# dkogan/libdogleg

Hardware: AMD Instinct MI355X
Metric: trust-region steps/sec (fp64) at fixed (Nmeas,Nstate,nnz) (higher is better)
Workload: dtype f64

## Files before the change

include/dlg_backend.h:

```cpp
#ifndef DLG_BACKEND_H
#define DLG_BACKEND_H

#include <stddef.h>

#ifdef __cplusplus
extern "C" {
#endif

typedef struct dlg_backend dlg_backend_t;

enum
{
  DLG_OK           = 0,
  DLG_ERR_HIP      = 1,
  DLG_ERR_ARG      = 2,
  DLG_ERR_STATE    = 3,
  DLG_ERR_NOMEM    = 4,
  DLG_ERR_NODEVICE = 5,
  DLG_ERR_COMM     = 6
};

enum { DLG_DENSE = 0, DLG_SPARSE = 1, DLG_DENSE_PRODUCTS = 2 };
enum { DLG_FLAG_JTJ_PACKED = 1, DLG_FLAG_JTJ_UPPER = 2 };
enum { DLG_KIND_CAUCHY_TO_EDGE = 0, DLG_KIND_GAUSSNEWTON = 1, DLG_KIND_INTERPOLATED = 2 };
// ... 21 lines not shown
int  dlg_partition_rows(dlg_backend_t* b, int* nrows, const int** rows);
int  dlg_point_gather_device(dlg_backend_t* b, int slot, const double* x_full_dev, const double* J_full_dev,
                             const int* colptr_host);
int  dlg_partition_stats(dlg_backend_t* b, long* stats, int nstats);
int  dlg_sparse_partition_probe(int N, int M, const int* colptr, const int* rowidx, int rank, int nranks,
                                long* stats, int nstats, char* row_owner);
int  dlg_rccl_unique_id(void* out128);
int  dlg_backend_init_rccl(dlg_backend_t* b, int rank, int nranks, const void* unique_id128);
int  dlg_backend_set_rccl(dlg_backend_t* b, void* nccl_comm);
int  dlg_backend_share_rccl(dlg_backend_t* b, dlg_backend_t* owner);
int  dlg_backend_comm_size(dlg_backend_t* b, int* nranks);
int  dlg_backend_has_rccl(dlg_backend_t* b);
int  dlg_backend_set_noop_comm(dlg_backend_t* b, int on);

int  dlg_run_steps(dlg_backend_t* b, int from, int to, int nsteps, int ncopy, const double* const* x_dev,
                   const double* const* J_dev, int first_copy, double trustregion, double lambda0,
                   double* out9, int* kind_out);

int  dlg_backend_reset(dlg_backend_t* b);
int  dlg_backend_device(dlg_backend_t* b);
int  dlg_sparse_pattern_matches(dlg_backend_t* b, const int* colptr, const int* rowidx);
int  dlg_sparse_drop_pattern(dlg_backend_t* b);

int  dlg_sparse_set_pattern(dlg_backend_t* b, const int* colptr, const int* rowidx);
int  dlg_sparse_stats(dlg_backend_t* b, long* nnz_JtJ_lower, long* nnz_L,
                      int* n_supernodes, int* n_levels, double* factor_flops);

int  dlg_sparse_region_probe(int N, int M, const int* colptr, const int* rowidx, int ncu, long* stats, int nstats);

int  dlg_sparse_schedule(dlg_backend_t* b, int* n_levels, int* persist_level0, int* persist_items);

int  dlg_sparse_leaf_rows_stats(dlg_backend_t* b, long* stats, int nstats);

int  dlg_sparse_symbolic_probe(int N, int M, const int* colptr, const int* rowidx, int row0,
                               int row1, long* stats, int nstats, int* perm_out);

int  dlg_point_set_p(dlg_backend_t* b, int slot, const double* p_host);
int  dlg_point_upload(dlg_backend_t* b, int slot, const double* x_host,
                      const double* J_host);
int  dlg_point_upload_products(dlg_backend_t* b, int slot, double norm2x,
                               const double* Jtx_host, const double* JtJ_host);
int  dlg_point_bind_device(dlg_backend_t* b, int slot, const double* x_dev,
                           const double* J_dev);
int  dlg_point_eval(dlg_backend_t* b, int slot, double* norm2_x, double* Jtx_absmax);
int  dlg_backend_set_speculation(dlg_backend_t* b, int on);
typedef void (*dlg_between_fn)(void* cookie);
int  dlg_backend_set_between(dlg_backend_t* b, dlg_between_fn fn, void* cookie);
int  dlg_backend_between_redone(dlg_backend_t* b);
int  dlg_point_eval_early(dlg_backend_t* b, int slot, const double* x_dev, const double* J_dev, int* done);
int  dlg_backend_set_defer_tail(dlg_backend_t* b, int on);
int  dlg_step_tail_pending(dlg_backend_t* b);
int  dlg_backend_ei_source(dlg_backend_t* b, int* from_solved_system, double* pivot_ratio);
int  dlg_step_tail(dlg_backend_t* b, double* expected_improvement);
int  dlg_backend_time_allreduce(dlg_backend_t* b, size_t count, int iters, double* us_each);

int  dlg_cauchy(dlg_backend_t* b, int slot, double* norm2_updateCauchy);

int  dlg_factorize(dlg_backend_t* b, int slot, double lambda, int* ok);

int  dlg_solve_gn(dlg_backend_t* b, int slot, double* norm2_updateGN);

int  dlg_gauss_newton(dlg_backend_t* b, int slot, double* lambda_io, double* norm2_updateGN);

int  dlg_cauchy_gauss_newton(dlg_backend_t* b, int slot, double* lambda_io, double* norm2_updateCauchy,
                             double* norm2_updateGN);

// ... 88 lines not shown
```

libdogleg_amd/capi.py:

```python
import ctypes as C
import os
import numpy as np

from .ctypes_defs import (Parameters2, CholmodSparse, Trace, TraceBuffer, BatchResult, BatchLoss, BatchBounds, JacobianReport, JacobianEntry,
                          CB_SPARSE, CB_DENSE, CB_PRODUCTS, dptr, iptr)

HERE = os.path.dirname(os.path.abspath(__file__))
LIB_PATH = os.environ.get("DLG_TEST_LIB") or os.path.join(HERE, "libdogleg_amd.so")

DLG_OK = 0
DLG_DENSE, DLG_SPARSE, DLG_DENSE_PRODUCTS = 0, 1, 2
FLAG_PACKED, FLAG_UPPER = 1, 2
KIND_CAUCHY, KIND_GN, KIND_INTERP = 0, 1, 2
VEC_P, VEC_X, VEC_JTX, VEC_CAUCHY, VEC_GN, VEC_STEP, VEC_J, VEC_X_OWN, VEC_J_OWN = range(9)

ALLREDUCE_FN = C.CFUNCTYPE(C.c_int, C.c_void_p, C.c_size_t, C.c_void_p)

BACKEND_SYMBOLS = [
    "dlg_last_error", "dlg_device_count", "dlg_backend_create", "dlg_backend_destroy",
    "dlg_backend_set_stream", "dlg_backend_get_stream", "dlg_backend_set_shard",
    "dlg_sparse_set_pattern", "dlg_sparse_stats", "dlg_sparse_schedule", "dlg_sparse_leaf_rows_stats", "dlg_point_set_p", "dlg_point_upload",
    "dlg_point_upload_products", "dlg_point_bind_device", "dlg_point_eval", "dlg_cauchy",
    "dlg_factorize", "dlg_solve_gn", "dlg_gauss_newton", "dlg_cauchy_gauss_newton", "dlg_make_step",
    "dlg_expected_improvement", "dlg_step", "dlg_take_step", "dlg_solve_with_factor",
    "dlg_point_download", "dlg_factor_download_dense", "dlg_point_device_ptr",
    "dlg_kernel_syrk_lower", "dlg_kernel_potrf_lower", "dlg_probe_mfma_f64", "dlg_probe_mfma_f64_clock", "dlg_probe_mfma_f64_waves",
    "dlg_probe_hbm_copy", "dlg_set_trace", "dlg_mem_alloc", "dlg_mem_free", "dlg_host_alloc",
    "dlg_host_free", "dlg_mem_upload",
    "dlg_mem_download", "dlg_mem_zero", "dlg_device_sync", "dlg_sparse_symbolic_probe",
    "dlg_backend_set_profiling", "dlg_backend_get_profile", "dlg_backend_get_profile_early",
    "dlg_backend_set_allreduce", "dlg_backend_set_partition", "dlg_partition_rows", "dlg_partition_stats",
    "dlg_sparse_partition_probe", "dlg_rccl_unique_id", "dlg_backend_init_rccl", "dlg_backend_set_rccl",
    "dlg_backend_comm_size", "dlg_backend_has_rccl", "dlg_backend_set_noop_comm", "dlg_solve_multi", "dlg_pseudoinverse_chunk", "dlg_backend_set_speculation", "dlg_backend_set_defer_tail", "dlg_step_tail",
    "dlg_step_tail_pending", "dlg_backend_ei_source", "dlg_backend_set_between", "dlg_backend_between_redone", "dlg_point_eval_early",
    "dlg_backend_share_rccl", "dlg_point_gather_device", "dlg_backend_reset", "dlg_backend_device",
    "dlg_sparse_pattern_matches", "dlg_sparse_drop_pattern", "dlg_sparse_region_probe", "dlg_run_steps", "dlg_backend_time_allreduce",
    "dlg_feature_leverage", "dlg_outlierness_factors", "dlg_leverage_query", "dlg_leverage_stats",
    "dlg_covariance_blocks", "dlg_marginal_variances", "dlg_covariance_stats", "dlg_covariance_plan_seconds",
    "dlg_covariance_plan_probe", "dlg_covariance_entries", "dlg_covariance_entries_stats", "dlg_covariance_entries_probe",
    "dlg_query_covariance", "dlg_query_covariance_stats", "dlg_query_covariance_plan_seconds", "dlg_query_covariance_plan_probe",
]
PROF_NAMES = ["K1_jtx", "K3K8_norm2Jv", "K4_kernel", "K4_total", "K5_factor", "K6_solve", "K7_step", "vec"]
DOGLEG_SYMBOLS = [
    "dogleg_getDefaultParameters", "dogleg_setMaxIterations",
    "dogleg_setTrustregionUpdateParameters", "dogleg_setDebug", "dogleg_setInitialTrustregion",
    "dogleg_setThresholds", "dogleg_optimize", "dogleg_optimize2", "dogleg_optimize_dense",
    "dogleg_optimize_dense2", "dogleg_optimize_dense_products", "dogleg_computeJtJfactorization",
    "dogleg_freeContext", "dogleg_testGradient", "dogleg_testGradient_dense",
    "dogleg_testGradient_dense_products",
    "dogleg_optimize_device2", "dogleg_amd_backend", "dogleg_amd_point_slot",
    "dogleg_amd_set_communicator", "dogleg_amd_set_allreduce", "dogleg_amd_clear_communicator",
    "dogleg_amd_rccl_unique_id", "dogleg_amd_rank", "dogleg_amd_release_cache",
    "dogleg_amd_id_file_publish", "dogleg_amd_id_file_wait", "dogleg_amd_last_solve_timing",
    "dogleg_getOutliernessFactors", "dogleg_markOutliers", "dogleg_reportOutliers",
# ... 30 lines not shown
                       "g.build()'` (there is no CPU fallback)")
    L = C.CDLL(LIB_PATH)
    D, I, V = C.POINTER(C.c_double), C.POINTER(C.c_int), C.c_void_p
    L.dlg_last_error.restype = C.c_char_p
    L.dlg_device_count.restype = C.c_int
    L.dlg_backend_create.argtypes = [C.POINTER(V), C.c_int, C.c_int, C.c_int, C.c_int, C.c_int, C.c_int]
    L.dlg_backend_destroy.argtypes = [V]
    L.dlg_backend_destroy.restype = None
    L.dlg_backend_set_stream.argtypes = [V, V]
    L.dlg_backend_get_stream.argtypes = [V]
    L.dlg_backend_get_stream.restype = V
    L.dlg_backend_set_shard.argtypes = [V, C.c_int, C.c_int, V, V]
    L.dlg_backend_set_allreduce.argtypes = [V, V, V]
    L.dlg_backend_set_speculation.argtypes = [V, C.c_int]
    L.dlg_backend_set_defer_tail.argtypes = [V, C.c_int]
    L.dlg_step_tail.argtypes = [V, C.POINTER(C.c_double)]
    L.dlg_step_tail_pending.argtypes = [V]
    L.dlg_backend_ei_source.argtypes = [V, I, D]
    L.dlg_backend_set_partition.argtypes = [V, C.c_int, C.c_int]
    L.dlg_partition_rows.argtypes = [V, I, C.POINTER(I)]
    L.dlg_partition_stats.argtypes = [V, C.POINTER(C.c_long), C.c_int]
    L.dlg_sparse_partition_probe.argtypes = [C.c_int, C.c_int, I, I, C.c_int, C.c_int, C.POINTER(C.c_long), C.c_int, C.c_char_p]
    L.dlg_rccl_unique_id.argtypes = [V]
    L.dlg_backend_init_rccl.argtypes = [V, C.c_int, C.c_int, V]
    L.dlg_backend_set_rccl.argtypes = [V, V]
    L.dlg_backend_comm_size.argtypes = [V, I]
    L.dlg_backend_has_rccl.argtypes = [V]
    L.dlg_backend_set_noop_comm.argtypes = [V, C.c_int]
    L.dlg_backend_get_profile_early.argtypes = [V, D, C.POINTER(C.c_long), C.c_int]
    L.dlg_sparse_set_pattern.argtypes = [V, I, I]
    L.dlg_sparse_stats.argtypes = [V, C.POINTER(C.c_long), C.POINTER(C.c_long), I, I, D]
    L.dlg_sparse_schedule.argtypes = [V, I, I, I]
    L.dlg_sparse_leaf_rows_stats.argtypes = [V, C.POINTER(C.c_long), C.c_int]
    L.dlg_point_set_p.argtypes = [V, C.c_int, D]
    L.dlg_point_upload.argtypes = [V, C.c_int, D, D]
    L.dlg_point_upload_products.argtypes = [V, C.c_int, C.c_double, D, D]
    L.dlg_point_bind_device.argtypes = [V, C.c_int, V, V]
    L.dlg_point_eval.argtypes = [V, C.c_int, D, D]
    L.dlg_cauchy.argtypes = [V, C.c_int, D]
    L.dlg_factorize.argtypes = [V, C.c_int, C.c_double, I]
    L.dlg_solve_gn.argtypes = [V, C.c_int, D]
    L.dlg_gauss_newton.argtypes = [V, C.c_int, D, D]
    L.dlg_cauchy_gauss_newton.argtypes = [V, C.c_int, D, D, D]
    L.dlg_make_step.argtypes = [V, C.c_int, C.c_int, C.c_int, C.c_double, D, D, D, D]
    L.dlg_step.argtypes = [V, C.c_int, C.c_int, C.c_int, C.c_double, D, D, D, D, D]
    L.dlg_take_step.argtypes = [V, C.c_int, C.c_int, C.c_double, D, D, D]
    L.dlg_solve_with_factor.argtypes = [V, C.c_int, D, D, C.c_int]
    L.dlg_solve_multi.argtypes = [V, C.c_int, D, D, C.c_int]
    L.dlg_pseudoinverse_chunk.argtypes = [V, C.c_int, C.c_int, C.c_int, D]
    L.dlg_feature_leverage.argtypes = [V, C.c_int, C.c_int, C.c_int, C.c_int, D]
    L.dlg_outlierness_factors.argtypes = [V, C.c_int, C.c_int, C.c_int, C.c_double, D]
    L.dlg_leverage_query.argtypes = [V, C.c_int, D, C.c_int, C.c_int, C.c_int, D]
    L.dlg_leverage_stats.argtypes = [V, C.c_int, C.POINTER(C.c_long), C.POINTER(C.c_long), I]
    L.dlg_covariance_blocks.argtypes = [V, C.c_int, C.c_int, I, I, I, I, D]
    L.dlg_marginal_variances.argtypes = [V, C.c_int, D]
    L.dlg_covariance_stats.argtypes = [V, C.POINTER(C.c_long), C.POINTER(C.c_long), I]
    L.dlg_covariance_plan_seconds.argtypes = [V]
    L.dlg_covariance_plan_seconds.restype = C.c_double
    L.dlg_covariance_plan_probe.argtypes = [C.c_int, C.c_int, I, I, C.c_int, I, I, I, I, I, C.POINTER(C.c_long), C.c_int]
    L.dlg_covariance_entries.argtypes = [V, C.c_int, C.c_long, I, I, D]
    L.dlg_covariance_entries_stats.argtypes = [V, D, C.POINTER(C.c_long), C.POINTER(C.c_long)]
    L.dlg_covariance_entries_probe.argtypes = [C.c_int, C.c_int, I, I, C.c_long, I, I, I, C.POINTER(C.c_long), C.c_int]
    if hasattr(L, "dlg_query_covariance"):
        L.dlg_query_covariance.argtypes = [V, C.c_int, C.c_int, I, I, I, D, C.c_int, D]
        L.dlg_query_covariance_stats.argtypes = [V, C.POINTER(C.c_long), C.POINTER(C.c_long), I]
        L.dlg_query_covariance_plan_seconds.argtypes = [V]
# ... 638 lines not shown

    def set_noop_comm(self, on=True):
        _ck(self.L.dlg_backend_set_noop_comm(self.h, 1 if on else 0), "set_noop_comm")

    def comm_size(self):
        n = C.c_int()
        _ck(self.L.dlg_backend_comm_size(self.h, C.byref(n)), "comm_size")
        return n.value

    def set_pattern(self, Jp, Ji):
        Jp = np.ascontiguousarray(Jp, dtype=np.int32)
        Ji = np.ascontiguousarray(Ji, dtype=np.int32)
        _ck(self.L.dlg_sparse_set_pattern(self.h, iptr(Jp), iptr(Ji)), "set_pattern")

    def stats(self):
        a, b = C.c_long(), C.c_long()
        c, d = C.c_int(), C.c_int()
        e = C.c_double()
        _ck(self.L.dlg_sparse_stats(self.h, C.byref(a), C.byref(b), C.byref(c), C.byref(d), C.byref(e)),
            "stats")
        return dict(nnz_JtJ_lower=a.value, nnz_L=b.value, n_supernodes=c.value, n_levels=d.value,
                    factor_flops=e.value)

    def schedule(self):
        a, b, c = C.c_int(), C.c_int(), C.c_int()
        _ck(self.L.dlg_sparse_schedule(self.h, C.byref(a), C.byref(b), C.byref(c)), "schedule")
        return dict(n_levels=a.value, persist_level0=b.value, persist_items=c.value)

    def leaf_rows_stats(self):
        v = (C.c_long * 4)()
        _ck(self.L.dlg_sparse_leaf_rows_stats(self.h, v, 4), "leaf_rows_stats")
        return dict(lean_launches=v[0], materialized=v[1], raw=bool(v[2]), lean_levels=v[3])

    def set_p(self, slot, p):
        p = np.ascontiguousarray(p, dtype=np.float64)
        _ck(self.L.dlg_point_set_p(self.h, slot, dptr(p)), "set_p")

    def upload(self, slot, x, J):
        x = np.ascontiguousarray(x, dtype=np.float64)
        J = np.ascontiguousarray(J, dtype=np.float64)
        self._keep = [x, J]
        _ck(self.L.dlg_point_upload(self.h, slot, dptr(x), dptr(J)), "upload")

    def upload_products(self, slot, norm2x, Jtx, JtJ):
        Jtx = np.ascontiguousarray(Jtx, dtype=np.float64)
        JtJ = np.ascontiguousarray(JtJ, dtype=np.float64)
        self._keep = [Jtx, JtJ]
        _ck(self.L.dlg_point_upload_products(self.h, slot, norm2x, dptr(Jtx), dptr(JtJ)), "upload")

    def bind_device(self, slot, x_ptr, J_ptr):
        _ck(self.L.dlg_point_bind_device(self.h, slot, C.c_void_p(x_ptr), C.c_void_p(J_ptr)), "bind")

    def eval(self, slot):
        a, b = C.c_double(), C.c_double()
        _ck(self.L.dlg_point_eval(self.h, slot, C.byref(a), C.byref(b)), "eval")
        return a.value, b.value

    def cauchy(self, slot):
        a = C.c_double()
        _ck(self.L.dlg_cauchy(self.h, slot, C.byref(a)), "cauchy")
        return a.value

    def factorize(self, slot, lam=0.0):
        ok = C.c_int()
        _ck(self.L.dlg_factorize(self.h, slot, lam, C.byref(ok)), "factorize")
        return bool(ok.value)
# ... 198 lines not shown
```

libdogleg_amd/csrc/sparse_internal.h:

```cpp
#pragma once
#include "dlg_internal.h"
#include "sparse_symbolic.h"
#include "sparse_region.h"
#include "leaf_rows_state.h"

namespace {
constexpr int JFL_SEG = 16;
constexpr int NV_CHUNK = 2048;

constexpr int TPB = 256;
constexpr int LDS_BUDGET = SYM_LDS_BUDGET;
constexpr int FAC_LDS_BUDGET = SYM_FAC_LDS_BUDGET;

__device__ __forceinline__ double wave_sum(double v)
{
#pragma unroll
  for(int o = 32; o > 0; o >>= 1) v += __shfl_down(v, o, 64);
  return v;
}

template <int NT, int U, class LoadF, class StoreF>
__device__ __forceinline__ void batched_copy(int total, int tid, LoadF ld, StoreF st)
{
  for(int base = 0; base < total; base += U*NT)
// ... 62 lines not shown
  double* top_scr = nullptr;
  const double* aug_rhs = nullptr;
  int *Jp = nullptr, *Ji = nullptr;
  int *gat_rows = nullptr, *gat_src = nullptr;
  int *nv_chunk = nullptr; int n_nv_chunks = 0;
  double *Lx = nullptr, *scr = nullptr, *ywork = nullptr, *asm_part = nullptr, *jtx_part = nullptr;
  int *d_info = nullptr, *h_info = nullptr;
  bool info_armed = false;
  bool zero_fail_seen = false; int64_t* leaf_diag = nullptr; int* leaf_diag_col = nullptr; int n_leaf_diag = 0;
  double* intact_Lx = nullptr; const double* intact_J = nullptr; int intact_slot = -1; double intact_lambda = 0.0;
  const double* fac_J = nullptr; int fac_slot = -1;
  bool fac_pending = false;
  size_t nnz_loc = 0;
  uint32_t* ar_idx = nullptr; double* ar_buf = nullptr; size_t ar_n = 0;
  FacLevels fac;
  std::vector<int> slv_lds, bwd_lds, bwd_nt, bwd_bd, bwd_pmx;
  int64_t* red_off = nullptr; int* red_len = nullptr; int* red_kind = nullptr; int64_t* red_dst = nullptr;
  int n_red_seg = 0; size_t red_n = 0; double* red_buf = nullptr;
  double* colmask = nullptr; int* sn_owner = nullptr;
  int64_t* augpos = nullptr;
  int *xl_sn = nullptr;
  double* held_Lx = nullptr; const double* held_aug = nullptr; double held_lambda = 0.0;
  LeafRowsState leaf_rows; std::vector<char> leaf_lean; double* leaf_rd = nullptr;
  double cur_lambda = 0.0;
  double *ms_scr = nullptr, *ms_y = nullptr; int ms_lds_f = 0, ms_lds_b = 0;
  typedef ReachPlan LevPlan;
  LevPlan lev[2];
  int* lev_iperm = nullptr; std::vector<int> lev_jp, lev_ji; int lev_lds = 0;
  double* Lx_spec = nullptr; hipEvent_t ev_spec = nullptr, ev_spec_fork = nullptr;
  bool spec_inflight = false, spec_valid = false; int spec_slot = -1; const double* spec_J = nullptr;
  int64_t touch_off = 0, touch_n = 0;
  int bw_level0 = 1 << 30, bw_lds = 0, bw_n = 0;
  SolveItem* slv_item_pr = nullptr; int* bwd_flag = nullptr; int bwd_epoch = 0; double* bwd_xh = nullptr;
  PrRegion top, lo; double* pr_acc = nullptr;
  int64_t* clr_off = nullptr; int64_t* clr_len = nullptr; int n_clr = 0; bool clr_partial_ok = false; double* lz_ok[2] = {nullptr, nullptr};
  int64_t* aug_of_var = nullptr; char* jf_listed = nullptr;
  int aug_fused_epoch = 0; const double* spec_aug_fused = nullptr;
  int* fin_flag = nullptr; int fin_epoch = 0, fin_side_owed = 0; bool fin_side_sched_ok = false; hipStream_t fin_main = nullptr;
  int bwd_xb_cap = 12288;
  double* diag_mm = nullptr; int n_diag_mm = 0;
  std::vector<void*> allocs;
};

int sparse_assemble(dlg_backend* b, int s, double lambda);
int sparse_partition_reduce(dlg_backend* b);
int sparse_assemble_speculative(dlg_backend* b, int s);
int sparse_eval_assemble(dlg_backend* b, int s, int* done);
int sparse_assemble_finish(dlg_backend* b);
int sparse_zero_spare(dlg_backend* b, hipStream_t ordered_for);
void sparse_spec_invalidate(dlg_backend* b, int s);
int sparse_factor_setup(dlg_backend* b);
int sparse_factor_levels(dlg_backend* b, int part = 0);
int sparse_solve_setup(dlg_backend* b);
```

libdogleg_amd/csrc/sparse_solve.hip:

```cpp
#include "sparse_internal.h"

namespace {
#ifdef DLG_FL_PROFILE
__device__ long long g_bw_prof[64*8];
__device__ long long g_bw_chain[256*8];
#define BW_STAMP(k) do { if(threadIdx.x == 0 && blockIdx.x == 0) g_bw_prof[(prof_lvl & 63)*8 + (k)] = clock64(); \
                         if(threadIdx.x == 0 && pr_flag && blockIdx.x < 256) g_bw_chain[blockIdx.x*8 + (k)] = wall_clock64(); } while(0)
#else
#define BW_STAMP(k)
#endif

__global__ void __launch_bounds__(TPB) k_solve_fwd_level(const int* __restrict__ lvl_sn,
                                                         const int* __restrict__ sn_c0,
                                                         const int* __restrict__ sn_rowptr,
                                                         const int64_t* __restrict__ sn_lx,
                                                         const int* __restrict__ sn_scr,
                                                         const int* __restrict__ rl_ptr,
                                                         const int* __restrict__ rl_pos,
                                                         const int* __restrict__ perm,
                                                         const double* __restrict__ Lx,
                                                         const double* __restrict__ rhs,
                                                         double* __restrict__ scr,
                                                         double* __restrict__ ywork)
{
// ... 40 lines not shown
      sum = wave_sum(sum);
      if(lane == 0) y[j] = rhs[perm[k]] - sum;
    }
  }
  __syncthreads();
  double yi = (tid < w) ? y[tid] : 0.0;
  for(int j = 0; j < w; j++)
  {
    if(tid == j) y[j] = yi / lds[j + j*ldp];
    __syncthreads();
    if(tid > j && tid < w) yi -= lds[tid + j*ldp]*y[j];
  }
  __syncthreads();
  for(int j = tid; j < w; j += TPB) ywork[c0 + j] = y[j];
  const int r = nrows - w - 1;
  double* u = scr + sn_scr[s];
  for(int i = tid; i < r; i += TPB)
  {
    double sum = 0.0;
#pragma unroll 8
    for(int j = 0; j < w; j++) sum += L[w + i + (size_t)j*nrows]*y[j];
    u[i] = sum;
  }
}
template <int BWD_NT, bool BD_ONLY>
__global__ void __launch_bounds__(BWD_NT, BD_ONLY ? 4 : 1) k_solve_bwd_level(const SolveItem* __restrict__ items,
                                                            const int* __restrict__ sn_rows,
                                                            const int* __restrict__ perm,
                                                            const double* __restrict__ Lx,
                                                            double* __restrict__ ywork,
                                                            double* __restrict__ out, int use_aug,
                                                            const int* __restrict__ sn_bd_col, int top_lds, int xb_cap,
                                                            int* pr_flag, int pr_epoch, const int* __restrict__ info, DlgHandoff ho,
                                                            double* xh, int xh_n, double* __restrict__ mm, int rows_raw)
{
  extern __shared__ __attribute__((aligned(16))) double lds[];
  __shared__ int s_skip;
  double dmin = 1e300, dmax = 0.0;
  if(threadIdx.x == 0) s_skip = *info != 0x7fffffff;
  constexpr int NW = BWD_NT/64;
  typedef const __attribute__((address_space(1))) double* gcd_t;
  typedef __attribute__((address_space(1))) double* gd_t;
  auto ldx = [&](const double* p) -> double { return pr_flag ? __hip_atomic_load((gcd_t)p, __ATOMIC_RELAXED, __HIP_MEMORY_SCOPE_AGENT) : *p; };
  constexpr unsigned long long X_EMPTY = 0x7FF8DEADBEEF0002ull;
  typedef __attribute__((address_space(1))) unsigned long long* gu_t;
  const bool xh_on = pr_flag != nullptr && xh != nullptr && ho.skew == 0;
  unsigned long long* xcur = reinterpret_cast<unsigned long long*>(xh) + (size_t)(pr_epoch & 1)*xh_n;
  auto put_xh = [&](int col, double v) {
    if(xh_on) __hip_atomic_store((gu_t)(xcur + col), (unsigned long long)__double_as_longlong(v), __ATOMIC_RELAXED, __HIP_MEMORY_SCOPE_AGENT); };
  auto take_xh = [&](int col) -> double {
    unsigned long long u; int spins = 0;
    while((u = __hip_atomic_load((gu_t)(xcur + col), __ATOMIC_RELAXED, __HIP_MEMORY_SCOPE_AGENT)) == X_EMPTY)
    { __builtin_amdgcn_s_sleep(1); if(++spins > ho.spins) { atomicOr(ho.status, DLG_HANDOFF_SOLVE); u = 0; break; } }
    return __longlong_as_double((long long)u); };

  const int prof_lvl = top_lds >> 8; (void)prof_lvl;
  top_lds &= 1;
  BW_STAMP(0);
  const SolveItem it = items[blockIdx.x];
  const int c0 = it.c0, w = it.w, nrows = it.nrows;
  if(xh_on && (int)threadIdx.x < w) reinterpret_cast<unsigned long long*>(xh)[(size_t)(1 - (pr_epoch & 1))*xh_n + c0 + threadIdx.x] = X_EMPTY;
  const int* rows = sn_rows + it.rowoff;
  const double* L = Lx + it.lx;
  const int tid = threadIdx.x, lane = tid & 63, wv = tid >> 6;
  const int r = nrows - w - 1;
  const int nblk = (w + 7) >> 3;
  const bool xb_lds = r <= xb_cap;
  double* xb = lds;
  double* xs = lds + (xb_lds ? ((r + 1) & ~1) : 0);
  double* T = xs + 256;
  double* rhs = T + nblk*64;
  double* xp = rhs + 16;
  double* Lt = xp + 8*256;
  const int ldt = w | 1;
  const int MW = (w + 15) & ~15;
  double* Mx = Lt + (top_lds ? w*ldt : 0);
  const int nmem = BD_ONLY ? max(it.nbd, 1) : it.nbd;
  const int myrow = (tid < r) ? rows[w + tid] : 0;
  double myrhs = 0.0; int myperm = 0;
  if(tid < w) { myrhs = use_aug ? L[(nrows - 1) + (size_t)tid*nrows] : ywork[c0 + tid]; myperm = perm[c0 + tid]; }
  constexpr bool LEAN = BWD_NT == 256;
  constexpr int MV_SLOTS = LEAN ? 20 : 24;
  const int mv_cols = min(BWD_NT, max(w, 64)), mv_parts = BWD_NT/mv_cols;
  const int mv_j = tid % mv_cols, mv_p = tid/mv_cols;
  const int mv_len = (r + mv_parts - 1)/mv_parts;
  const int mv_i0 = mv_p*mv_len, mv_i1 = min(r, mv_i0 + mv_len);
  const bool mv_thread = mv_len <= MV_SLOTS && xb_lds;
  const bool mv_on = mv_thread && mv_j < w && mv_p < mv_parts;
  const double* mv_L = L + (size_t)min(mv_j, w - 1)*nrows + w;
  double mv[MV_SLOTS];
  {
    typedef double bw_v2d __attribute__((ext_vector_type(2)));
    typedef bw_v2d bw_v2d_u __attribute__((aligned(8)));
#pragma unroll
    for(int q = 0; q < MV_SLOTS; q += 2)
    {
      if(mv_on && mv_i0 + q + 1 < mv_i1) { const bw_v2d t = *reinterpret_cast<const bw_v2d_u*>(mv_L + mv_i0 + q); mv[q] = t.x; mv[q + 1] = t.y; }
      else { mv[q] = (mv_on && mv_i0 + q < mv_i1) ? mv_L[mv_i0 + q] : 0.0; mv[q + 1] = 0.0; }
    }
  }
  if(!BD_ONLY)
  for(int e = tid; e < (nmem > 0 ? 0 : nblk*64); e += BWD_NT)
  {
    const int j0 = (e >> 6)*8, a = (e >> 3) & 7, b = e & 7;
    const bool valid = a >= b && j0 + a < w;
    double v = valid ? L[(j0 + a) + (size_t)(j0 + b)*nrows] : 0.0;
    if(a == b && valid) { dmin = fmin(dmin, v); dmax = fmax(dmax, v); }
    if(a == b) v = valid ? 1.0/v : 1.0;
    T[e] = v;
  }
  if(!BD_ONLY && top_lds && nmem == 0)
  {
    const int cp_rows = min(BWD_NT, (w + 63) & ~63), cp_ng = BWD_NT/cp_rows, cp_g = tid/cp_rows;
// ... 8 lines not shown
      }
  }
  double Lm[8][8];
  int m0 = 0, nbm = 0;
  if(nmem > 0 && tid < nmem)
  {
    if(it.rsv > 0) { m0 = tid*it.rsv; nbm = it.rsv; }
    else
    {
      const int* mcol = sn_bd_col + it.bd0;
      m0 = mcol[tid]; nbm = ((tid + 1 < nmem) ? mcol[tid + 1] : w) - m0;
    }
  }
  if(nmem > 0)
  {
#pragma unroll
    for(int a = 0; a < 8; a++)
#pragma unroll
      for(int b = 0; b <= a; b++) Lm[a][b] = (a < nbm) ? L[(m0 + a) + (size_t)(m0 + b)*nrows] : (a == b ? 1.0 : 0.0);
    if(mm)
    {
#pragma unroll
      for(int a = 0; a < 8; a++) if(a < nbm) { dmin = fmin(dmin, Lm[a][a]); dmax = fmax(dmax, Lm[a][a]); }
    }
  }
  if(mm && (nmem > 0 ? 64*wv < nmem : wv < nblk))
  {
#pragma unroll
    for(int o = 32; o > 0; o >>= 1) { dmin = fmin(dmin, __shfl_down(dmin, o, 64)); dmax = fmax(dmax, __shfl_down(dmax, o, 64)); }
    if(lane == 0) { mm[(8*blockIdx.x + wv)*2] = dmin; mm[(8*blockIdx.x + wv)*2 + 1] = dmax; }
  }
  BW_STAMP(1);
  const bool premul = it.rsv != 0 && !BD_ONLY && nmem == 0 && pr_flag != nullptr && it.pflag >= 0;
  if(premul)
  {
    __syncthreads();
    double ti[8];
    const bool ton = tid < 8*nblk;
    if(ton)
    {
      const double* Tb = T + (tid >> 3)*64;
      const int c = tid & 7;
      double Lb[8][8];
#pragma unroll
      for(int a = 0; a < 8; a++)
#pragma unroll
        for(int b2 = 0; b2 <= a; b2++) Lb[a][b2] = Tb[a*8 + b2];
#pragma unroll
      for(int i = 0; i < 8; i++)
      {
        double v = 0.0;
#pragma unroll
        for(int k = 0; k < i; k++) v -= (k >= c) ? Lb[i][k]*ti[k] : 0.0;
        ti[i] = (i == c) ? Lb[i][i] : ((i > c) ? v*Lb[i][i] : 0.0);
      }
    }
    __syncthreads();
    if(ton)
    {
      double* Tb = T + (tid >> 3)*64;
      const int c = tid & 7;
#pragma unroll
      for(int i = 0; i < 8; i++) if(i >= c) Tb[i*8 + c] = ti[i];
    }
    __syncthreads();
    if(tid < w)
    {
      const double* Lc = L + (size_t)tid*nrows;
      const int wl = w - 1, b0 = (tid >> 3) + 1;
      double cur[8], nxt[8];
#pragma unroll
      for(int a = 0; a < 8; a++) { cur[a] = Lc[min(8*min(b0, nblk - 1) + a, wl)]; nxt[a] = Lc[min(8*min(b0 + 1, nblk - 1) + a, wl)]; }
      for(int blk = b0; blk < nblk; blk++)
      {
        double far[8];
#pragma unroll
        for(int a = 0; a < 8; a++) far[a] = Lc[min(8*min(blk + 2, nblk - 1) + a, wl)];
        const double* Tb = T + blk*64;
#pragma unroll
        for(int b2 = 0; b2 < 8; b2++)
        {
          double m = Tb[b2*8]*cur[0];
#pragma unroll
          for(int a = 1; a <= b2; a++) m += Tb[b2*8 + a]*cur[a];
          Mx[(blk*8 + b2)*MW + tid] = m;
        }
#pragma unroll
        for(int a = 0; a < 8; a++) { cur[a] = nxt[a]; nxt[a] = far[a]; }
      }
    }
  }
  if(tid < 256) xs[tid] = 0.0;
  const bool by_value = xh_on && xb_lds;
  if(pr_flag && !by_value)
  {
    if(tid == 0 && it.pflag >= 0)
    {
      int spins = 0;
      while(__hip_atomic_load(pr_flag + it.pflag, __ATOMIC_RELAXED, __HIP_MEMORY_SCOPE_AGENT) != pr_epoch + ho.skew)
      {
        __builtin_amdgcn_s_sleep(1);
        if(++spins > ho.spins) { atomicOr(ho.status, DLG_HANDOFF_SOLVE); break; }
      }
    }
    __syncthreads();
  }
  if(by_value)
  {
    if(tid < r) xb[tid] = take_xh(myrow);
    for(int i = tid + BWD_NT; i < r; i += BWD_NT) xb[i] = take_xh(rows[w + i]);
  }
  else if(xb_lds)
  {
    if(tid < r) xb[tid] = ldx(ywork + myrow);
    for(int i = tid + BWD_NT; i < r; i += BWD_NT) xb[i] = ldx(ywork + rows[w + i]);
  }
  __syncthreads();
  if(s_skip)
  {
    if(tid < w) put_xh(c0 + tid, 0.0);
    if(pr_flag && tid == 0) __hip_atomic_store(pr_flag + blockIdx.x, pr_epoch, __ATOMIC_RELAXED, __HIP_MEMORY_SCOPE_AGENT);
    return;
  }
  BW_STAMP(2);
// ... 24 lines not shown
    for(int q = 0; q < MV_SLOTS; q++) acc += mv[q]*((mv_i0 + q < mv_i1) ? xb[mv_i0 + q] : 0.0);
    if(mv_on) xp[mv_p*256 + mv_j] = acc;
  }
  else
  {
    for(int e = 256 + tid; e < mv_parts*256; e += BWD_NT) xp[e] = 0.0;
    for(int jg = 4*wv; jg < w; jg += 4*NW)
    {
      const double* Lj = L + (size_t)jg*nrows + w;
      const int nc = min(4, w - jg);
      double acc[4] = {0.0, 0.0, 0.0, 0.0};
#pragma unroll 2
      for(int i = lane; i < r; i += 64)
      {
        const double x = xb_lds ? xb[i] : ldx(ywork + rows[w + i]);
#pragma unroll
        for(int c = 0; c < 4; c++) acc[c] += ((c < nc) ? Lj[i + (size_t)c*nrows] : 0.0)*x;
      }
#pragma unroll
      for(int c = 0; c < 4; c++)
      {
        const double sum = wave_sum(acc[c]);
        if(lane == 0 && c < nc) xp[jg + c] = sum;
      }
    }
  }
  double Lz[4][4];
  if(LEAN && rows_raw)
  {
#pragma unroll
    for(int a = 0; a < 4; a++)
#pragma unroll
      for(int b = 0; b <= a; b++) Lz[a][b] = (tid < nmem && a < nbm) ? L[(m0 + a) + (size_t)(m0 + b)*nrows] : (a == b ? 1.0 : 0.0);
  }
  __syncthreads();
  BW_STAMP(3);
  if(tinv_on)
  {
    double* Tb = T + (tid >> 3)*64;
    const int c = tid & 7;
#pragma unroll
    for(int i = 0; i < 8; i++) if(i >= c) Tb[i*8 + c] = tinv[i];
  }
  if(nmem > 0)
  {
    if(tid < w)
    {
      double sum = 0.0;
      for(int p = 0; p < mv_parts; p++) sum += xp[p*256 + tid];
      if(rows_raw) { xs[tid] = sum; xp[tid] = myrhs; }
      else xs[tid] = myrhs - sum;
    }
    __syncthreads();
    if(rows_raw && tid < nmem)
    {
      double z[4];
#pragma unroll
      for(int a = 0; a < 4; a++)
      {
        double v = (a < nbm) ? xs[m0 + a] : 0.0;
#pragma unroll
        for(int b = 0; b < a; b++) v -= (LEAN ? Lz[a][b] : Lm[a][b])*z[b];
        z[a] = v/(LEAN ? Lz[a][a] : Lm[a][a]);
      }
#pragma unroll
      for(int a = 0; a < 4; a++) if(a < nbm) xs[m0 + a] = xp[m0 + a] - z[a];
// ... 10 lines not shown
        }
    }
    else if(tid < nmem)
    {
      double xk[8];
#pragma unroll
      for(int a = 7; a >= 0; a--)
      {
        double v = (a < nbm) ? xs[m0 + a] : 0.0;
#pragma unroll
        for(int b = a + 1; b < 8; b++) v -= Lm[b][a]*xk[b];
        xk[a] = v/Lm[a][a];
      }
#pragma unroll
      for(int a = 0; a < 8; a++) if(a < nbm) xs[m0 + a] = xk[a];
    }
    __syncthreads();
    if(tid < w)
    {
      put_xh(c0 + tid, xs[tid]);
      if(pr_flag) __hip_atomic_store((gd_t)(ywork + c0 + tid), xs[tid], __ATOMIC_RELAXED, __HIP_MEMORY_SCOPE_AGENT);
      else ywork[c0 + tid] = xs[tid];
      out[myperm] = xs[tid];
    }
    if(pr_flag)
    {
      asm volatile("s_waitcnt vmcnt(0)" ::: "memory");
      __syncthreads();
      if(tid == 0) __hip_atomic_store(pr_flag + blockIdx.x, pr_epoch, __ATOMIC_RELAXED, __HIP_MEMORY_SCOPE_AGENT);
    }
    return;
  }
  if(BD_ONLY) return;
  if(tid >= ((8*nblk + 63) & ~63)) return;
  double xi = 0.0;
  if(tid < w)
  {
    double sum = 0.0;
    for(int p = 0; p < mv_parts; p++) sum += xp[p*256 + tid];
    xi = myrhs - sum;
  }
  if(premul)
  {
    const int own = tid & 7;
    for(int blk = nblk - 1; blk >= 0; blk--)
    {
      const int j0 = 8*blk;
      double* rh = rhs + 8*(blk & 1);
      if(tid >= j0 && tid < j0 + 8) rh[tid - j0] = xi;
      const double* Mb = (tid < j0) ? Mx + (size_t)blk*8*MW + tid : T + blk*64 + own;
      const int mst = (tid < j0) ? MW : 8;
      double mb[8];
#pragma unroll
      for(int b2 = 0; b2 < 8; b2++) mb[b2] = Mb[b2*mst];
      asm volatile("s_waitcnt lgkmcnt(0)\n\ts_barrier" ::: "memory");
      double r8[8];
#pragma unroll
      for(int b2 = 0; b2 < 8; b2 += 2)
      {
        const double2 rr = *reinterpret_cast<const double2*>(rh + b2);
        r8[b2] = rr.x; r8[b2 + 1] = rr.y;
      }
      double v = mb[0]*r8[0];
#pragma unroll
      for(int b2 = 1; b2 < 8; b2++) v += mb[b2]*r8[b2];
      if(tid < j0) xi -= v;
// ... 95 lines not shown
}

__global__ void __launch_bounds__(TPB) k_touch(const double2* __restrict__ p, size_t n2, double* __restrict__ sink)
{
  double acc = 0.0;
  for(size_t i = blockIdx.x*(size_t)TPB + threadIdx.x; i < n2; i += (size_t)gridDim.x*TPB)
  { const double2 v = p[i]; acc += v.x + v.y; }
  if(acc == 1.2345678e300) sink[0] = acc;
}
__global__ void __launch_bounds__(TPB) k_mask_vec(double* __restrict__ v, const double* __restrict__ mask, int n,
                                                  const double* __restrict__ extra)
{
  const int i = blockIdx.x*TPB + threadIdx.x;
  if(i < n) v[i] *= mask[i];
  if(extra && i == 0) v[n] = *extra;
}

}

#ifdef DLG_FL_PROFILE
extern "C" void dlg_bw_profile_dump(int nlevels)
{
  long long h[64*8];
  hipDeviceSynchronize();
  {
    std::vector<long long> c(256*8);
    hipMemcpyFromSymbol(c.data(), HIP_SYMBOL(g_bw_chain), sizeof(long long)*c.size());
    long long t0 = 0;
    for(int g = 0; g < 256; g++) if(c[g*8] && (t0 == 0 || c[g*8] < t0)) t0 = c[g*8];
    for(int g = 0; g < 256 && g < (getenv("DLG_FL_DUMP_ALL") ? 256 : 24); g++)
    {
      const long long* q = &c[g*8];
      if(q[5] == 0) continue;
      fprintf(stderr, "   bwd wg %3d: start %6lld loads issued %6lld parent there + x gathered %6lld mat-vec %6lld sweep %6lld published %6lld (10 ns)\n",
              g, q[0] - t0, q[1] - t0, q[2] - t0, q[3] - t0, q[4] - t0, q[5] - t0);
    }
  }
  hipMemcpyFromSymbol(h, HIP_SYMBOL(g_bw_prof), sizeof(h));
  for(int l = 0; l < nlevels && l < 64; l++)
    fprintf(stderr, "bwd level %2d: issue %6lld  gather+barrier %6lld  matvec %6lld  solve %6lld  store %6lld cycles | to first barrier %6lld, in it %6lld, rest of the loop %6lld\n", l,
            h[l*8+1] - h[l*8], h[l*8+2] - h[l*8+1], h[l*8+3] - h[l*8+2], h[l*8+4] - h[l*8+3], h[l*8+5] - h[l*8+4],
            h[l*8+6] - h[l*8+3], h[l*8+7] - h[l*8+6], h[l*8+4] - h[l*8+7]);
}
#endif
int sparse_touch_factor(dlg_backend* b, hipStream_t st)
{
  SparseSym* Y = b->sym;
  if(!Y || !Y->touch_n) return DLG_OK;
  const int nwg = b->knobs.touch_wg;
  hipLaunchKernelGGL(k_touch, dim3(nwg), dim3(TPB), 0, st, reinterpret_cast<const double2*>(Y->Lx + Y->touch_off),
                     (size_t)Y->touch_n/2, Y->ywork);
  DLG_LAUNCH_CHECK();
  return DLG_OK;
}
static SolveItem solve_item(const SymHost& H, int s)
{
  SolveItem it;
  it.c0 = H.sn_c0[s]; it.w = H.sn_c0[s+1] - H.sn_c0[s]; it.nrows = H.sn_rowptr[s+1] - H.sn_rowptr[s];
  it.rowoff = H.sn_rowptr[s]; it.lx = H.sn_lx[s]; it.bd0 = H.sn_bd_ptr[s]; it.nbd = H.sn_bd_ptr[s+1] - H.sn_bd_ptr[s];
  it.pflag = -1; it.rsv = 0;
  return it;
}

int sparse_solve_setup(dlg_backend* b)
{
  SparseSym* Y = b->sym;
  const SymHost& H = Y->H;
  const long xb_cap = env_int("DOGLEG_AMD_BWD_XB_CAP", 12288);
// ... 40 lines not shown
    {
      const int s = H.xl_sn[k];
      SolveItem& it = items[k];
      it = solve_item(H, s);
      it.rsv = Y->bwd_pmx[H.sn_level[s]] ? 1 : 0;
      if(it.nbd > 0)
      {
        const int* mc = &H.sn_bd_col[it.bd0];
        const int wd0 = (it.nbd > 1 ? mc[1] : it.w) - mc[0];
        bool same = mc[0] == 0;
        for(int m = 0; m < it.nbd && same; m++) if(((m + 1 < it.nbd) ? mc[m+1] : it.w) - mc[m] != wd0 || mc[m] != m*wd0) same = false;
        it.rsv = same ? wd0 : 0;
      }
    }
    DLG_CHECK(upload(Y->slv_item, items)); Y->allocs.push_back(Y->slv_item);
    std::vector<double> none(16*std::max<size_t>(items.size(), 1));
    for(size_t i = 0; i < none.size(); i += 2) { none[i] = 1e300; none[i + 1] = 0.0; }
    DLG_CHECK(upload(Y->diag_mm, none)); Y->allocs.push_back(Y->diag_mm);
    Y->n_diag_mm = 8*(int)items.size();
  }
  {
    int64_t lo = -1, hi = 0;
    for(int i = H.lvl_ptr[0]; i < H.lvl_ptr[1]; i++)
    {
      const int s = H.lvl_sn[i];
      const int64_t a = H.sn_lx[s], e = a + (int64_t)(H.sn_rowptr[s+1] - H.sn_rowptr[s])*(H.sn_c0[s+1] - H.sn_c0[s]);
      if(lo < 0 || a < lo) lo = a;
      if(e > hi) hi = e;
    }
    Y->touch_off = 0; Y->touch_n = 0;
    if(lo >= 0 && H.nlevels >= 3 && hi - lo >= (1 << 20) && (hi - lo)*8 <= (int64_t)200 << 20)
    { Y->touch_off = lo & ~(int64_t)1; Y->touch_n = (hi - Y->touch_off) & ~(int64_t)1; }
  }
  Y->bw_level0 = H.nlevels; Y->bw_n = 0;
  if(!getenv("DOGLEG_AMD_NO_PERSIST") && H.nlevels >= 2)
  {
    int ncu = 256;
    { int dev = 0; if(hipGetDevice(&dev) == hipSuccess) (void)hipDeviceGetAttribute(&ncu, hipDeviceAttributeMultiprocessorCount, dev); }
    const int cap = env_int("DOGLEG_AMD_PERSIST_MAX", 2*ncu);
    int total = 0, l0 = H.nlevels, ldsb = 0;
    for(int l = H.nlevels - 1; l >= 1; l--)
    {
      const int n = H.xl_ptr[l+1] - H.xl_ptr[l];
      if(n == 0 || total + n > cap || Y->bwd_nt[l] != 512 || Y->bwd_bd[l]) break;
      total += n; l0 = l; ldsb = std::max(ldsb, Y->bwd_lds[l]);
    }

    if(H.nlevels - l0 >= 2)
    {
      std::vector<SolveItem> items;
      std::vector<int> pos(H.nsn, -1);
      for(int l = H.nlevels - 1; l >= l0; l--)
        for(int k = H.xl_ptr[l]; k < H.xl_ptr[l+1]; k++)
        {
          const int s = H.xl_sn[k];
          SolveItem it = solve_item(H, s);
          it.rsv = Y->bwd_pmx[l] ? 1 : 0;
          if(it.nbd > 0) it.rsv = 0;
          if(it.nrows - it.w - 1 > 0)
          {
            const int prow = H.sn_rows[H.sn_rowptr[s] + it.w];
            const int ps = H.col_sn[prow];
            it.pflag = pos[ps];
            if(it.pflag < 0) { dlg_set_error("internal error: the parent of supernode %d is not part of the persistent backward launch", s); return DLG_ERR_ARG; }
          }
          pos[s] = (int)items.size();
          items.push_back(it);
        }
      Y->bw_level0 = l0; Y->bw_n = (int)items.size(); Y->bw_lds = std::max(ldsb, 84*1024);
      DLG_CHECK(upload(Y->slv_item_pr, items)); Y->allocs.push_back(Y->slv_item_pr);
      std::vector<unsigned long long> empty(2*(size_t)H.N, 0x7FF8DEADBEEF0002ull);
      DLG_HIP(hipMalloc(&Y->bwd_xh, sizeof(double)*empty.size())); Y->allocs.push_back(Y->bwd_xh);
      DLG_HIP(hipMemcpy(Y->bwd_xh, empty.data(), sizeof(double)*empty.size(), hipMemcpyHostToDevice));
      DLG_HIP(hipMalloc(&Y->bwd_flag, sizeof(int)*items.size())); Y->allocs.push_back(Y->bwd_flag);
      DLG_HIP(hipMemsetAsync(Y->bwd_flag, 0, sizeof(int)*items.size(), b->stream));
      Y->bwd_epoch = 0;
    }
  }
  for(int l = 0; l < H.nlevels; l++)
    if(Y->leaf_lean[l] && (l >= Y->bw_level0 || !Y->bwd_bd[l])) Y->leaf_lean[l] = 0;
  for(const void* k : { (const void*)&k_solve_fwd_level, (const void*)&k_solve_bwd_level<256, false>,
                        (const void*)&k_solve_bwd_level<256, true>, (const void*)&k_solve_bwd_level<512, false> })
    DLG_HIP(hipFuncSetAttribute(k, hipFuncAttributeMaxDynamicSharedMemorySize, LDS_BUDGET));
  return DLG_OK;
}

static double* bwd_diag_mm(const dlg_backend* b, int l)
{
  const SparseSym* Y = b->sym;
  return (Y->diag_mm && !b->knobs.ei_jpass) ? Y->diag_mm + 16*(size_t)Y->H.xl_ptr[l] : (double*)nullptr;
}
static void launch_bwd_level(dlg_backend* b, int nt, bool bd, int grid, int lds, const SolveItem* items, double* out, int use_aug,
                             int l, int* flag, int epoch, double* xh, int nxh)
{
  SparseSym* Y = b->sym;
  double* mm = bwd_diag_mm(b, l);
  const int rows_raw = (Y->leaf_lean[l] && Y->leaf_rows.raw(Y->Lx)) ? 1 : 0;
#define DLG_BW_LAUNCH(...) hipLaunchKernelGGL(HIP_KERNEL_NAME(k_solve_bwd_level<__VA_ARGS__>), dim3(grid), dim3(nt), lds, b->stream, \
                                              items, Y->sn_rows, Y->perm, Y->Lx, Y->ywork, out, use_aug, Y->sn_bd_col, 256*l, Y->bwd_xb_cap, \
                                              flag, epoch, Y->d_info, dlg_handoff(b, 1 << 21), xh, nxh, mm, rows_raw)
  if(nt == 256 && bd) DLG_BW_LAUNCH(256, true);
  else if(nt == 256) DLG_BW_LAUNCH(256, false);
  else { nt = 512; DLG_BW_LAUNCH(512, false); }
#undef DLG_BW_LAUNCH
}

int sparse_solve(dlg_backend* b, const double* rhs, double* out)
{
  SparseSym* Y = b->sym;
  if(!Y) { dlg_set_error("dlg_sparse_set_pattern must be called first"); return DLG_ERR_STATE; }
  const SymHost& H = Y->H;
  hipStream_t st = b->stream;
  const int use_aug = (Y->aug_rhs != nullptr && Y->aug_rhs == rhs) ? 1 : 0;
  if(H.part_nranks > 1 && !use_aug)
  { dlg_set_error("with a subtree partition only the right-hand side that rode along with the factorisation (Jt x) can be solved for"); return DLG_ERR_STATE; }
  if(!use_aug) DLG_CHECK(sparse_leaf_rows_materialize(b));
  for(int l = 0; l < H.nlevels && !use_aug; l++)
  {
    const int n = H.xl_ptr[l+1] - H.xl_ptr[l];
    if(n > 0)
      hipLaunchKernelGGL(k_solve_fwd_level, dim3(n), dim3(TPB), Y->slv_lds[l], st, Y->xl_sn + H.xl_ptr[l],
                         Y->sn_c0, Y->sn_rowptr, Y->sn_lx, Y->sn_scr, Y->rl_ptr, Y->rl_pos, Y->perm,
                         Y->Lx, rhs, Y->scr, Y->ywork);
  }
  if(H.part_nranks > 1) DLG_HIP(hipMemsetAsync(out, 0, sizeof(double)*(size_t)H.N, st));
  int ltop = H.nlevels - 1;
  if(Y->bw_level0 < H.nlevels)
  {
    DlgRegionTurn turn(b);
    launch_bwd_level(b, 512, false, Y->bw_n, Y->bw_lds, Y->slv_item_pr, out, use_aug, Y->bw_level0, Y->bwd_flag, ++Y->bwd_epoch, Y->bwd_xh, H.N);
    ltop = Y->bw_level0 - 1;
  }
  for(int l = ltop; l >= 0; l--)
  {
    const int n = H.xl_ptr[l+1] - H.xl_ptr[l];
    if(n > 0) launch_bwd_level(b, Y->bwd_nt[l], Y->bwd_bd[l], n, Y->bwd_lds[l], Y->slv_item + H.xl_ptr[l], out, use_aug, l, (int*)nullptr, 0, (double*)nullptr, 0);
  }
// ... 14 lines not shown
```

Baseline: 1844.

## Precompute explicit inverse of diagonal block in persistent backward solve

For persistent backward-solve supernodes of width at most 128 that are already premultiplied, the kernel now builds the full inverse of the triangular diagonal block in LDS while it waits for the parent. Once the parent's values arrive, the triangular sweep becomes a dense mat-vec using cross-lane reads. This shortens the critical path between the parent publishing and the child publishing, at the cost of extra flops and LDS work before the wait, a slightly different rounding order, and a global atomic counter plus a stats API added for diagnostics.

Result: no change. 1865 (median of 6 runs) (+1.1%).

```diff
diff --git a/include/dlg_backend.h b/include/dlg_backend.h
--- a/include/dlg_backend.h
+++ b/include/dlg_backend.h
@@ -77,6 +77,8 @@
 
 int  dlg_sparse_leaf_rows_stats(dlg_backend_t* b, long* stats, int nstats);
 
+int  dlg_sparse_bwd_form_stats(dlg_backend_t* b, long* stats, int nstats);
+
 int  dlg_sparse_symbolic_probe(int N, int M, const int* colptr, const int* rowidx, int row0,
                                int row1, long* stats, int nstats, int* perm_out);
 
diff --git a/libdogleg_amd/capi.py b/libdogleg_amd/capi.py
--- a/libdogleg_amd/capi.py
+++ b/libdogleg_amd/capi.py
@@ -19,7 +19,7 @@
 BACKEND_SYMBOLS = [
     "dlg_last_error", "dlg_device_count", "dlg_backend_create", "dlg_backend_destroy",
     "dlg_backend_set_stream", "dlg_backend_get_stream", "dlg_backend_set_shard",
-    "dlg_sparse_set_pattern", "dlg_sparse_stats", "dlg_sparse_schedule", "dlg_sparse_leaf_rows_stats", "dlg_point_set_p", "dlg_point_upload",
+    "dlg_sparse_set_pattern", "dlg_sparse_stats", "dlg_sparse_schedule", "dlg_sparse_leaf_rows_stats", "dlg_sparse_bwd_form_stats", "dlg_point_set_p", "dlg_point_upload",
     "dlg_point_upload_products", "dlg_point_bind_device", "dlg_point_eval", "dlg_cauchy",
     "dlg_factorize", "dlg_solve_gn", "dlg_gauss_newton", "dlg_cauchy_gauss_newton", "dlg_make_step",
     "dlg_expected_improvement", "dlg_step", "dlg_take_step", "dlg_solve_with_factor",
@@ -116,6 +116,7 @@
     L.dlg_sparse_stats.argtypes = [V, C.POINTER(C.c_long), C.POINTER(C.c_long), I, I, D]
     L.dlg_sparse_schedule.argtypes = [V, I, I, I]
     L.dlg_sparse_leaf_rows_stats.argtypes = [V, C.POINTER(C.c_long), C.c_int]
+    L.dlg_sparse_bwd_form_stats.argtypes = [V, C.POINTER(C.c_long), C.c_int]
     L.dlg_point_set_p.argtypes = [V, C.c_int, D]
     L.dlg_point_upload.argtypes = [V, C.c_int, D, D]
     L.dlg_point_upload_products.argtypes = [V, C.c_int, C.c_double, D, D]
@@ -820,6 +821,11 @@
         _ck(self.L.dlg_sparse_leaf_rows_stats(self.h, v, 4), "leaf_rows_stats")
         return dict(lean_launches=v[0], materialized=v[1], raw=bool(v[2]), lean_levels=v[3])
 
+    def bwd_form_stats(self):
+        v = (C.c_long * 5)()
+        _ck(self.L.dlg_sparse_bwd_form_stats(self.h, v, 5), "bwd_form_stats")
+        return dict(product=v[0], premul=v[1], product_taken=v[2], product_long=v[3], product_wide=v[4])
+
     def set_p(self, slot, p):
         p = np.ascontiguousarray(p, dtype=np.float64)
         _ck(self.L.dlg_point_set_p(self.h, slot, dptr(p)), "set_p")
diff --git a/libdogleg_amd/csrc/sparse_internal.h b/libdogleg_amd/csrc/sparse_internal.h
--- a/libdogleg_amd/csrc/sparse_internal.h
+++ b/libdogleg_amd/csrc/sparse_internal.h
@@ -118,6 +118,7 @@
   int64_t touch_off = 0, touch_n = 0;
   int bw_level0 = 1 << 30, bw_lds = 0, bw_n = 0;
   SolveItem* slv_item_pr = nullptr; int* bwd_flag = nullptr; int bwd_epoch = 0; double* bwd_xh = nullptr;
+  unsigned long long* bwd_form_cnt = nullptr; int bwd_n_product = 0, bwd_n_premul = 0, bwd_n_product_long = 0, bwd_n_product_wide = 0;
   PrRegion top, lo; double* pr_acc = nullptr;
   int64_t* clr_off = nullptr; int64_t* clr_len = nullptr; int n_clr = 0; bool clr_partial_ok = false; double* lz_ok[2] = {nullptr, nullptr};
   int64_t* aug_of_var = nullptr; char* jf_listed = nullptr;
diff --git a/libdogleg_amd/csrc/sparse_solve.hip b/libdogleg_amd/csrc/sparse_solve.hip
--- a/libdogleg_amd/csrc/sparse_solve.hip
+++ b/libdogleg_amd/csrc/sparse_solve.hip
@@ -96,7 +96,8 @@
                                                             double* __restrict__ out, int use_aug,
                                                             const int* __restrict__ sn_bd_col, int top_lds, int xb_cap,
                                                             int* pr_flag, int pr_epoch, const int* __restrict__ info, DlgHandoff ho,
-                                                            double* xh, int xh_n, double* __restrict__ mm, int rows_raw)
+                                                            double* xh, int xh_n, double* __restrict__ mm, int rows_raw,
+                                                            unsigned long long* form_cnt)
 {
   extern __shared__ __attribute__((aligned(16))) double lds[];
   __shared__ int s_skip;
@@ -143,6 +144,9 @@
   const int myrow = (tid < r) ? rows[w + tid] : 0;
   double myrhs = 0.0; int myperm = 0;
   if(tid < w) { myrhs = use_aug ? L[(nrows - 1) + (size_t)tid*nrows] : ywork[c0 + tid]; myperm = perm[c0 + tid]; }
+  double prhs = 0.0, prhs1 = 0.0;
+  if(BWD_NT == 512 && !BD_ONLY && it.rsv == 2 && nmem == 0 && lane < w) prhs = use_aug ? L[(nrows - 1) + (size_t)lane*nrows] : ywork[c0 + lane];
+  if(BWD_NT == 512 && !BD_ONLY && it.rsv == 2 && nmem == 0 && lane + 64 < w) prhs1 = use_aug ? L[(nrows - 1) + (size_t)(lane + 64)*nrows] : ywork[c0 + lane + 64];
   constexpr bool LEAN = BWD_NT == 256;
   constexpr int MV_SLOTS = LEAN ? 20 : 24;
   const int mv_cols = min(BWD_NT, max(w, 64)), mv_parts = BWD_NT/mv_cols;
@@ -217,6 +221,7 @@
   }
   BW_STAMP(1);
   const bool premul = it.rsv != 0 && !BD_ONLY && nmem == 0 && pr_flag != nullptr && it.pflag >= 0;
+  const bool product = BWD_NT == 512 && premul && it.rsv == 2 && w <= 128;
   if(premul)
   {
     __syncthreads();
@@ -274,7 +279,45 @@
         for(int a = 0; a < 8; a++) { cur[a] = nxt[a]; nxt[a] = far[a]; }
       }
     }
-  }
+    if(product)
+    {
+      if(form_cnt && tid == 0) atomicAdd(form_cnt, 1ull);
+      const int ra = __builtin_amdgcn_readfirstlane(wv);
+      const int cc0 = min(lane, MW - 1), cc1 = min(lane + 64, MW - 1);
+      __syncthreads();
+      for(int c = lane; c < MW; c += 64)
+        for(int I = 0; I <= (c >> 3) && I < nblk; I++)
+          Mx[(8*I + ra)*MW + c] = ((c >> 3) == I) ? T[I*64 + ra*8 + (c & 7)] : 0.0;
+      __syncthreads();
+      auto dot = [&](const double* Mr, int cc, int kb0, int kb1) -> double {
+        double s[4] = {0.0, 0.0, 0.0, 0.0};
+#pragma unroll 2
+        for(int kb = kb0; kb < kb1; kb++)
+        {
+          double m[8], l[8];
+#pragma unroll
+          for(int i = 0; i < 8; i += 2)
+          {
+            const double2 mm2 = *reinterpret_cast<const double2*>(Mr + 8*kb + i);
+            m[i] = mm2.x; m[i + 1] = mm2.y;
+          }
+#pragma unroll
+          for(int i = 0; i < 8; i++) l[i] = Mx[(8*kb + i)*MW + cc];
+#pragma unroll
+          for(int i = 0; i < 8; i++) s[i & 3] -= m[i]*l[i];
+        }
+        return (s[0] + s[1]) + (s[2] + s[3]); };
+      for(int I = 1; I < nblk; I++)
+      {
+        double* Mr = Mx + (8*I + ra)*MW;
+        const double s0 = dot(Mr, cc0, 0, I), s1 = dot(Mr, cc1, 8, I);
+        if(lane < 8*I) Mr[lane] = s0;
+        if(lane + 64 < 8*I) Mr[lane + 64] = s1;
+        __syncthreads();
+      }
+    }
+  }
+  BW_STAMP(6);
   if(tid < 256) xs[tid] = 0.0;
   const bool by_value = xh_on && xb_lds;
   if(pr_flag && !by_value)
@@ -365,6 +408,21 @@
     for(int a = 0; a < 4; a++)
 #pragma unroll
       for(int b = 0; b <= a; b++) Lz[a][b] = (tid < nmem && a < nbm) ? L[(m0 + a) + (size_t)(m0 + b)*nrows] : (a == b ? 1.0 : 0.0);
+  }
+  double li0[8], li1[8], li2[8];
+#pragma unroll
+  for(int a = 0; a < 8; a++) { li0[a] = 0.0; li1[a] = 0.0; li2[a] = 0.0; }
+  if(product)
+  {
+    const int ra = __builtin_amdgcn_readfirstlane(wv);
+    const int cc0 = min(lane, MW - 1), cc1 = min(lane + 64, MW - 1);
+#pragma unroll
+    for(int a = 0; a < 8; a++) li0[a] = Mx[min(8*ra + a, w - 1)*MW + cc0];
+    if(w > 64)
+    {
+#pragma unroll
+      for(int a = 0; a < 8; a++) { const int q1 = min(64 + 8*ra + a, w - 1)*MW; li1[a] = Mx[q1 + cc0]; li2[a] = Mx[q1 + cc1]; }
+    }
   }
   __syncthreads();
   BW_STAMP(3);
@@ -441,6 +499,59 @@
     return;
   }
   if(BD_ONLY) return;
+  if(product)
+  {
+    const bool wide = w > 64;
+    const int pl = mv_parts - 1;
+    auto masked = [&](double v, int p) -> double { return __longlong_as_double(__double_as_longlong(v) & (p <= pl ? -1ll : 0ll)); };
+    double pt[8];
+#pragma unroll
+    for(int p = 0; p < 8; p++) pt[p] = xp[min(p, pl)*256 + lane];
+    double sum0 = 0.0, sum1 = 0.0;
+#pragma unroll
+    for(int p = 0; p < 8; p++) sum0 += masked(pt[p], p);
+    if(wide)
+    {
+#pragma unroll
+      for(int p = 0; p < 8; p++) pt[p] = xp[min(p, pl)*256 + 64 + lane];
+#pragma unroll
+      for(int p = 0; p < 8; p++) sum1 += masked(pt[p], p);
+    }
+    const double rr0 = (lane < w) ? prhs - sum0 : 0.0, rr1 = (lane + 64 < w) ? prhs1 - sum1 : 0.0;
+    const int ra = __builtin_amdgcn_readfirstlane(wv);
+    auto from_lane = [&](double v, int l) -> double {
+      return __hiloint2double(__builtin_amdgcn_readlane(__double2hiint(v), l), __builtin_amdgcn_readlane(__double2loint(v), l)); };
+    double v0 = 0.0, v1 = 0.0;
+#pragma unroll
+    for(int a = 0; a < 8; a++) v0 += li0[a]*from_lane(rr0, 8*ra + a);
+    if(wide)
+    {
+#pragma unroll
+      for(int a = 0; a < 8; a++) { const double rk = from_lane(rr1, 8*ra + a); v0 += li1[a]*rk; v1 += li2[a]*rk; }
+    }
+    double* part = xp + 128;
+    part[ra*256 + lane] = v0;
+    if(wide) part[ra*256 + 64 + lane] = v1;
+    asm volatile("s_waitcnt lgkmcnt(0)\n\ts_barrier" ::: "memory");
+    if(tid >= (wide ? 128 : 64)) return;
+#pragma unroll
+    for(int p = 0; p < 8; p++) pt[p] = part[p*256 + tid];
+    double xi = 0.0;
+#pragma unroll
+    for(int p = 0; p < 8; p++) xi += pt[p];
+    BW_STAMP(4);
+    if(tid < w)
+    {
+      put_xh(c0 + tid, xi);
+      __hip_atomic_store((gd_t)(ywork + c0 + tid), xi, __ATOMIC_RELAXED, __HIP_MEMORY_SCOPE_AGENT);
+      out[myperm] = xi;
+    }
+    asm volatile("s_waitcnt vmcnt(0)" ::: "memory");
+    __syncthreads();
+    if(tid == 0) __hip_atomic_store(pr_flag + blockIdx.x, pr_epoch, __ATOMIC_RELAXED, __HIP_MEMORY_SCOPE_AGENT);
+    BW_STAMP(5);
+    return;
+  }
   if(tid >= ((8*nblk + 63) & ~63)) return;
   double xi = 0.0;
   if(tid < w)
@@ -602,8 +713,8 @@
     {
       const long long* q = &c[g*8];
       if(q[5] == 0) continue;
-      fprintf(stderr, "   bwd wg %3d: start %6lld loads issued %6lld parent there + x gathered %6lld mat-vec %6lld sweep %6lld published %6lld (10 ns)\n",
-              g, q[0] - t0, q[1] - t0, q[2] - t0, q[3] - t0, q[4] - t0, q[5] - t0);
+      fprintf(stderr, "   bwd wg %3d: start %6lld loads issued %6lld prepared %6lld parent there + x gathered %6lld mat-vec %6lld sweep %6lld published %6lld (10 ns)\n",
+              g, q[0] - t0, q[1] - t0, q[6] - t0, q[2] - t0, q[3] - t0, q[4] - t0, q[5] - t0);
     }
   }
   hipMemcpyFromSymbol(h, HIP_SYMBOL(g_bw_prof), sizeof(h));
@@ -710,7 +821,8 @@
     if(lo >= 0 && H.nlevels >= 3 && hi - lo >= (1 << 20) && (hi - lo)*8 <= (int64_t)200 << 20)
     { Y->touch_off = lo & ~(int64_t)1; Y->touch_n = (hi - Y->touch_off) & ~(int64_t)1; }
   }
-  Y->bw_level0 = H.nlevels; Y->bw_n = 0;
+  Y->bw_level0 = H.nlevels; Y->bw_n = 0; Y->bwd_n_product = 0; Y->bwd_n_premul = 0; Y->bwd_n_product_long = 0; Y->bwd_n_product_wide = 0;
+  const bool product_ok = !getenv("DOGLEG_AMD_NO_PRODUCT");
   if(!getenv("DOGLEG_AMD_NO_PERSIST") && H.nlevels >= 2)
   {
     int ncu = 256;
@@ -742,6 +854,11 @@
             it.pflag = pos[ps];
             if(it.pflag < 0) { dlg_set_error("internal error: the parent of supernode %d is not part of the persistent backward launch", s); return DLG_ERR_ARG; }
           }
+          if(it.rsv == 1 && it.pflag >= 0 && product_ok && it.w <= 128 && total <= ncu) it.rsv = 2;
+          if(it.pflag >= 0 && it.nbd == 0) { Y->bwd_n_product += it.rsv == 2; Y->bwd_n_premul += it.rsv == 1; }
+          const int rb = it.nrows - it.w - 1;
+          if(it.rsv == 2 && (rb > 24*(512/std::max(it.w, 64)) || rb > xb_cap)) Y->bwd_n_product_long++;
+          if(it.rsv == 2 && it.w > 64) Y->bwd_n_product_wide++;
           pos[s] = (int)items.size();
           items.push_back(it);
         }
@@ -752,6 +869,8 @@
       DLG_HIP(hipMemcpy(Y->bwd_xh, empty.data(), sizeof(double)*empty.size(), hipMemcpyHostToDevice));
       DLG_HIP(hipMalloc(&Y->bwd_flag, sizeof(int)*items.size())); Y->allocs.push_back(Y->bwd_flag);
       DLG_HIP(hipMemsetAsync(Y->bwd_flag, 0, sizeof(int)*items.size(), b->stream));
+      DLG_HIP(hipMalloc(&Y->bwd_form_cnt, sizeof(unsigned long long))); Y->allocs.push_back(Y->bwd_form_cnt);
+      DLG_HIP(hipMemsetAsync(Y->bwd_form_cnt, 0, sizeof(unsigned long long), b->stream));
       Y->bwd_epoch = 0;
     }
   }
@@ -776,11 +895,26 @@
   const int rows_raw = (Y->leaf_lean[l] && Y->leaf_rows.raw(Y->Lx)) ? 1 : 0;
 #define DLG_BW_LAUNCH(...) hipLaunchKernelGGL(HIP_KERNEL_NAME(k_solve_bwd_level<__VA_ARGS__>), dim3(grid), dim3(nt), lds, b->stream, \
                                               items, Y->sn_rows, Y->perm, Y->Lx, Y->ywork, out, use_aug, Y->sn_bd_col, 256*l, Y->bwd_xb_cap, \
-                                              flag, epoch, Y->d_info, dlg_handoff(b, 1 << 21), xh, nxh, mm, rows_raw)
+                                              flag, epoch, Y->d_info, dlg_handoff(b, 1 << 21), xh, nxh, mm, rows_raw, flag ? Y->bwd_form_cnt : nullptr)
   if(nt == 256 && bd) DLG_BW_LAUNCH(256, true);
   else if(nt == 256) DLG_BW_LAUNCH(256, false);
   else { nt = 512; DLG_BW_LAUNCH(512, false); }
 #undef DLG_BW_LAUNCH
+}
+
+extern "C" int dlg_sparse_bwd_form_stats(dlg_backend_t* b, long* stats, int nstats)
+{
+  if(!b || !b->sym || !stats) { dlg_set_error("no symbolic analysis yet"); return DLG_ERR_STATE; }
+  const SparseSym* Y = b->sym;
+  unsigned long long taken = 0;
+  if(Y->bwd_form_cnt)
+  {
+    DLG_HIP(hipStreamSynchronize(b->stream));
+    DLG_HIP(hipMemcpy(&taken, Y->bwd_form_cnt, sizeof(taken), hipMemcpyDeviceToHost));
+  }
+  const long v[] = { Y->bwd_n_product, Y->bwd_n_premul, (long)taken, Y->bwd_n_product_long, Y->bwd_n_product_wide };
+  for(int i = 0; i < nstats && i < 5; i++) stats[i] = v[i];
+  return DLG_OK;
 }
 
 int sparse_solve(dlg_backend* b, const double* rhs, double* out)
```
